# avaneev/avir

Measured on AMD Instinct MI355X. Metric: Mpixels/sec (output) for 4K->8K RGBA resize, higher is better.
Workload: dtype f32; 1 GPU; cfg3: 3840x2160->7680x4320 RGBA float32, avir::CImageResizer<>(16), k=0, default params, frame resident in HBM

## Files before the change

avir_amd/csrc/up2.hip:

```cpp

#include "plan.h"
#include "up2_chunks.h"
#include <algorithm>
#include <string.h>
#include <stdlib.h>
#include <stdio.h>
#include <type_traits>

namespace avirhip {

typedef float f4 __attribute__(( ext_vector_type( 4 )));
typedef float f2 __attribute__(( ext_vector_type( 2 )));
typedef unsigned u2 __attribute__(( ext_vector_type( 2 )));

#ifndef U2_TW
#define U2_TW 64
#endif
#define U2_NT ( U2_TW * 2 )
#ifndef U2_RB
#define U2_RB 8
#endif
#ifndef U2_HS
#define U2_HS 4
#endif
#define U2_SW ( U2_TW / 2 + 18 )
#define U2_CW ( U2_TW / 2 + 12 )

struct Up2Params
{
	const float* src; long src_ss; int sw, sh;
	int rmin, rmax;
	float* dst; long dst_ss; int dst_row0; int nw, nh;
	int srow_lo, srow_hi;
	int nstrips, chunk0, nchunks;
	int cq, nlong;
	void* ibase; int istride_b; int ich;
#ifdef U2_DBG
	int dbg;
	unsigned long long* clk;
#endif
	const float* coef;
};

typedef float f8 __attribute__(( ext_vector_type( 8 )));
typedef float f16 __attribute__(( ext_vector_type( 16 )));
#define U2_PAIRED 64

__device__ __forceinline__ f2 splat( const float c )
{
	f2 r; r.x = c; r.y = c; return( r );
}

struct Taps
{
	f16 a, b, c;
	f8 d;
	__device__ __forceinline__ f2 pr( const f16& v, int i ) const
		{ f2 r; r.x = v[ 2 * i ]; r.y = v[ 2 * i + 1 ]; return( r ); }
	__device__ __forceinline__ f2 f( int i ) const { return( pr( a, i )); }
	__device__ __forceinline__ f2 fe( int i ) const
		{ return( i < 4 ? pr( a, 4 + i ) : pr( b, i - 4 )); }
	__device__ __forceinline__ f2 fo( int i ) const
	{
		if( i < 8 ) return( pr( c, i ));
		f2 r; r.x = d[ 2 * ( i - 8 )]; r.y = d[ 2 * ( i - 8 ) + 1 ];
		return( r );
	}
};

__device__ __forceinline__ const float* sgpr_ptr( const float* p )
{
	const unsigned long long a = (unsigned long long) p;
	const unsigned lo = __builtin_amdgcn_readfirstlane( (unsigned) a );
	const unsigned hi = __builtin_amdgcn_readfirstlane( (unsigned) ( a >> 32 ));
	return( (const float*) (( (unsigned long long) hi << 32 ) | lo ));
}

__device__ __forceinline__ Taps load_taps( const float* p0 )
{
	const float* const p = sgpr_ptr( p0 );
	Taps t;
	asm volatile( "s_load_dwordx16 %0, %4, 0x0\n\t"
		"s_load_dwordx16 %1, %4, 0x40\n\t"
		"s_load_dwordx16 %2, %4, 0x80\n\t"
		"s_load_dwordx8 %3, %4, 0xc0\n\t"
		AVIRHIP_WAITCNT_LGKM( 0 )
		: "=&s"( t.a ), "=&s"( t.b ), "=&s"( t.c ), "=&s"( t.d )
		: "s"( p ) : "memory" );
	return( t );
}

struct TapsI
{
	f8 a;
	f4 b;
	__device__ __forceinline__ f2 fe( int i ) const
		{ return( splat( i < 8 ? a[ i ] : b[ i - 8 ])); }
};

__device__ __forceinline__ TapsI load_taps_i( const float* p0 )
{
	const float* const p = sgpr_ptr( p0 );
	TapsI t;
	asm volatile( "s_load_dwordx8 %0, %2, 0x10\n\t"
		"s_load_dwordx4 %1, %2, 0x30\n\t"
		AVIRHIP_WAITCNT_LGKM( 0 )
		: "=&s"( t.a ), "=&s"( t.b ) : "s"( p ) : "memory" );
	return( t );
}

struct TapsE
{
	f16 a;
	__device__ __forceinline__ f2 f( int i ) const { return( splat( a[ i ])); }
	__device__ __forceinline__ f2 fe( int i ) const { return( splat( a[ 4 + i ])); }
};

__device__ __forceinline__ TapsE load_taps_e( const float* p0 )
{
	const float* const p = sgpr_ptr( p0 );
	TapsE t;
	asm volatile( "s_load_dwordx16 %0, %1, 0x0\n\t"
		AVIRHIP_WAITCNT_LGKM( 0 )
		: "=&s"( t.a ) : "s"( p ) : "memory" );
	return( t );
}

__device__ __forceinline__ f4 load_f4( const float* p0 )
{
	const float* const p = sgpr_ptr( p0 );
	f4 t;
	asm volatile( "s_load_dwordx4 %0, %1, 0x0\n\t" AVIRHIP_WAITCNT_LGKM( 0 )
		: "=&s"( t ) : "s"( p ) : "memory" );
	return( t );
}

__device__ __forceinline__ f8 load_f8( const float* p0 )
{
	const float* const p = sgpr_ptr( p0 );
	f8 t;
	asm volatile( "s_load_dwordx8 %0, %1, 0x0\n\t" AVIRHIP_WAITCNT_LGKM( 0 )
		: "=&s"( t ) : "s"( p ) : "memory" );
	return( t );
}

__device__ __forceinline__ f4 tmul( const f2 t, const f4 v )
{
	const f2 lo = t * v.lo;
	const f2 hi = t * v.hi;
	return( __builtin_shufflevector( lo, hi, 0, 1, 2, 3 ));
}

__device__ __forceinline__ int fresh_tid( const int wave )
{
	int l;
	asm volatile( "v_mbcnt_lo_u32_b32 %0, -1, 0\n\t"
		"v_mbcnt_hi_u32_b32 %0, -1, %0" : "=v"( l ));
	return( l + wave * 64 );
}

__device__ __forceinline__ int clampi( int i, int hi )
{
	return( i < 0 ? 0 : ( i > hi ? hi : i ));
}

#if U2_TW == 32
#define U2_SYNC() __builtin_amdgcn_fence( __ATOMIC_RELEASE, "wavefront" ); \
	__builtin_amdgcn_wave_barrier(); \
	__builtin_amdgcn_fence( __ATOMIC_ACQUIRE, "wavefront" )
#else
#define U2_SYNC() do { AVIRHIP_BARRIER_DRAIN(); __syncthreads(); } while( 0 )

#define U2_PRIO_H 0
#define U2_PRIO_V 1

__device__ __forceinline__ void u2_setprio( const int p )
{
	if( p == 0 ) __builtin_amdgcn_s_setprio( 0 );
	else if( p == 1 ) __builtin_amdgcn_s_setprio( 1 );
	else if( p == 2 ) __builtin_amdgcn_s_setprio( 2 );
	else __builtin_amdgcn_s_setprio( 3 );
}
#endif

#ifdef U2_DBG
#define U2_ON( bit ) ( !( P.dbg & ( bit )))
#define U2_ABL_H1( k ) ( !( P.dbg & 16 ) || ( k ) < 2 || wave == 0 )
#define U2_ABL_TAIL() ( !( P.dbg & 32 ) || abl_tail == 0 )
#else
#define U2_ON( bit ) true
#define U2_ABL_H1( k ) true
#define U2_ABL_TAIL() true
#endif

#ifndef U2_STAUX
#define U2_STAUX 2
#endif

#ifndef U2_LDAUX
#define U2_LDAUX 0
#endif

#define U2_TPL ( U2_RB * ( U2_TW / 2 ) + 8 )

#ifndef U2_H2PB
#define U2_H2PB 4
#endif

template< bool VT, int IO = 0, int SRC = 0 >
__global__ void __launch_bounds__( U2_NT )
__attribute__(( amdgpu_waves_per_eu( 4, 4 ))) k_up2( const Up2Params P )
{
	static_assert( IO == 0 || VT, "the fused output stage lives in the VT form" );
	static_assert( SRC == 0 || VT, "raw sources live in the VT form" );
	constexpr int SESZ = SRC / 10;
	constexpr int SCH = SRC % 10;
	constexpr int PXB = ( SRC != 0 ? SESZ * SCH : 16 );
	constexpr int ESZ = ( IO == 1 || IO == 4 ? 1 : ( IO == 2 || IO == 5 ? 2 : 4 ));
	__shared__ __attribute__(( aligned( 16 ))) f4 sS[ U2_RB * U2_SW ];
	__shared__ __attribute__(( aligned( 16 ))) f4 sC[ U2_RB * U2_CW ];
	__shared__ __attribute__(( aligned( 16 ))) f4 sT[ U2_TPL * 2 - 8 ];

#ifdef U2_DBG
	const unsigned long long dbg_c0 = clock64();
	const unsigned long long dbg_w0 = wall_clock64();

	if( P.dbg & ( 2048 | 4096 ))
	{
		const int slot = ( P.dbg & 2048 ? (( blockIdx.x >> 8 ) & 1 ) * 4 :
			( blockIdx.x >> 8 ) & 7 );

		for( int i = 0; i < slot; i++ )
		{
			__builtin_amdgcn_s_sleep( 25 );
		}
	}
#endif
	const int nwg = gridDim.x;
	const int b = blockIdx.x;
	const int xcd = b & 7;
	const int qd = nwg >> 3;
	const int rm = nwg & 7;
	const int item = ( xcd < rm ? xcd * ( qd + 1 ) :
		rm * ( qd + 1 ) + ( xcd - rm ) * qd ) + ( b >> 3 );

	const int strip = item / P.nchunks;
	const int chunk = P.chunk0 + item - strip * P.nchunks;
	const int tid = threadIdx.x;
	const int hf = tid & 1;
	const int col = tid >> 1;

	const int qx0 = strip * ( U2_TW / 2 );
	const int qy0 = up2_chunk_first( chunk, P.cq, P.nlong );
	const int qy1 = min( qy0 + up2_chunk_rows( chunk, P.cq, P.nlong ),
		P.nh >> 1 );
	const int u0 = qy0 - 9;
	const int nsteps = qy1 - qy0 + 18;
	const int xo = qx0 * 2 + col;
	const int ylo = max( qy0 * 2, P.srow_lo );
	const int yhi = min( qy1 * 2, P.srow_hi );
	const bool xok = ( xo < P.nw );
	const bool strip_full = ( qx0 * 2 + U2_TW <= P.nw );
	const int dlane_b = ( xo * 4 + hf * 2 ) * 4;
	const int drow_b = ( IO != 0 ? P.istride_b :
		(int) P.dst_ss * 4 );
	const int srow_b = (int) P.src_ss * ( SRC != 0 ? 1 : 4 );

	const int ubase = max( u0, P.rmin );
	const char* const sbase = (const char*) P.src + (long) ubase * srow_b;
	const int rsh = ( SRC != 0 ? (int) ( (unsigned long long) sbase & 3 ) : 0 );
	const __amdgpu_buffer_rsrc_t rsrc = __builtin_amdgcn_make_buffer_rsrc(
		(void*) ( sbase - rsh ), 0, ( SRC != 0 ?
		( rsh + ( P.rmax - ubase ) * srow_b + P.sw * PXB + 3 ) & ~3 : 0x7fffffff ),
		0x00020000 );
	const __amdgpu_buffer_rsrc_t rdst = __builtin_amdgcn_make_buffer_rsrc(
		(void*) ( P.dst + (long) ( qy0 * 2 - P.dst_row0 ) * P.dst_ss ), 0,
		0x7fffffff, 0x00020000 );

	f2 tw[ 8 ];
	f2 cw[ VT ? 1 : 16 ];
	f2 ea[ VT ? 12 : 1 ];
	f2 oa[ VT ? 12 : 1 ];

#pragma unroll
	for( int i = 0; i < 8; i++ ) tw[ i ] = (f2) 0.0f;
#pragma unroll
	for( int i = 0; i < ( VT ? 1 : 16 ); i++ ) cw[ i ] = (f2) 0.0f;
#pragma unroll
	for( int i = 0; i < ( VT ? 12 : 1 ); i++ ) ea[ i ] = oa[ i ] = (f2) 0.0f;

	constexpr int RPI0 = U2_NT / U2_SW;
	constexpr int CN0 = U2_RB * U2_CW;
	unsigned pkA = 0;
	unsigned pkB = 0;
	unsigned pkC = 0;
	unsigned pkD = 0;
	int pvoff = -1;
	int dlv = 0;
	int dlv2 = 0;

	if constexpr( VT )
	{
		typedef __attribute__(( address_space( 3 ))) void* lp;
		auto la = []( const void* q ) -> unsigned
			{ return( (unsigned) (unsigned long long) (lp) q ); };

		{
			const int r = tid / U2_SW;
			const int sx = clampi( qx0 - 9 + ( tid - r * U2_SW ), P.sw - 1 );
			pvoff = ( tid < RPI0 * U2_SW ? r * srow_b + sx * PXB + rsh : -1 );
		}

		if constexpr( IO != 0 )
		{
			dlv = ( xo < P.nw && hf * 2 < P.ich ?
				( xo * P.ich + hf * 2 ) * ESZ : (int) 0x80000000u );
			dlv2 = ( xo < P.nw && hf * 2 + 1 < P.ich ?
				( xo * P.ich + hf * 2 + 1 ) * ESZ : (int) 0x80000000u );
		}
		else
		{
			dlv = ( xo < P.nw ? ( xo * 4 + hf * 2 ) * 4 : (int) 0x80000000u );
		}

		{
			constexpr int LS = ( U2_HS == 4 ? 2 : 1 );
			const int hr = ( tid >> 6 ) * 4 + (( tid >> ( 1 + LS )) & 3 );
			const int hq = (( tid >> ( 3 + LS )) & ( 8 / U2_HS - 1 )) * 4 * U2_HS +
				(( tid >> 1 ) & ( U2_HS - 1 ));

			pkA = la( (const f2*) &sC[ hr * U2_CW + hq ] + hf ) |
				( la( (const f2*) sT + ((( col & 1 ) * U2_TPL + ( col >> 1 )) * 2 +
				hf )) << 16 );
			pkD = la( &sC[ tid ]) |
				( la( (const f2*) &sT[ hr * ( U2_TW / 2 ) + hq ] + hf ) << 16 );
		}

		unsigned ha[ 3 ], hd = 0;
#pragma unroll
		for( int k = 0; k < 3; k++ )
		{
			const int i = min( tid + k * U2_NT, CN0 - 1 );
			const int r = (int) ((unsigned) i / U2_CW );
			ha[ k ] = la( &sS[ i + r * ( U2_SW - U2_CW )]);
			hd = la( &sC[ i ]);
		}

		pkB = ha[ 0 ] | ( ha[ 1 ] << 16 );
		pkC = ha[ 2 ] | ( hd << 16 );
		asm volatile( "" : "+v"( pkA ), "+v"( pkB ), "+v"( pkC ), "+v"( pkD ),
			"+v"( pvoff ), "+v"( dlv ));

		if constexpr( IO != 0 )
		{
			asm volatile( "" : "+v"( dlv2 ));
		}
	}

	typedef const __attribute__(( address_space( 3 ))) f4* lds_cf4;
	typedef __attribute__(( address_space( 3 ))) f4* lds_f4;
	typedef const __attribute__(( address_space( 3 ))) f2* lds_cf2;
	typedef __attribute__(( address_space( 3 ))) f2* lds_f2;
	auto lo16 = []( const unsigned v ) -> unsigned
	{
		unsigned r;
		asm volatile( "v_and_b32 %0, 0xffff, %1" : "=v"( r ) : "v"( v ));
		return( r );
	};
	auto hi16 = []( const unsigned v ) -> unsigned
	{
		unsigned r;
		asm volatile( "v_lshrrev_b32 %0, 16, %1" : "=v"( r ) : "v"( v ));
		return( r );
	};

	constexpr int RPI = U2_NT / U2_SW;
	constexpr int NDMA = U2_RB / RPI;
	static_assert( RPI >= 1 && U2_RB % RPI == 0, "S tile / DMA geometry" );

	typedef __attribute__(( address_space( 3 ))) void* ldsptr;
	const int wave = __builtin_amdgcn_readfirstlane( tid >> 6 );
	const int wave_b = wave * 1024;

	auto raw_off = [&]( const int k, const int ub ) -> int
	{
		if( ub >= P.rmin && ub + U2_RB <= P.rmax + 1 )
		{
			return( pvoff >= 0 ? pvoff + ( ub - ubase + k * RPI ) * srow_b : -1 );
		}

		const int tid = fresh_tid( wave );
		const int pr_r = tid / U2_SW;
		const int pr_sx = clampi( qx0 - 9 + ( tid - pr_r * U2_SW ), P.sw - 1 );
		const int sy = min( max( ub + k * RPI + pr_r, P.rmin ), P.rmax );

		return( tid < RPI * U2_SW ? ( sy - ubase ) * srow_b + pr_sx * PXB + rsh :
			-1 );
	};

	auto land_raw = [&]( const int ub )
	{
		typedef const __attribute__(( address_space( 3 ))) unsigned* lds_cu;
		unsigned d0[ NDMA ], d1[ NDMA ];
		int off[ NDMA ];
		const int lw = ( threadIdx.x & 63 ) * 4;
#pragma unroll
		for( int k = 0; k < NDMA; k++ )
		{
			off[ k ] = raw_off( k, ub );
			const char* const st = (const char*) sS + k * RPI * U2_SW * 16 +
				wave_b + lw;
			d0[ k ] = *(lds_cu) (const void*) st;
			d1[ k ] = *(lds_cu) (const void*) ( st + 256 );
		}

		asm volatile( "s_waitcnt lgkmcnt(0)" ::: "memory" );
#pragma unroll
		for( int k = 0; k < NDMA; k++ )
		{
			if( off[ k ] >= 0 )
			{
				const unsigned sh = (unsigned) off[ k ] & 3u;
				const unsigned lo = __builtin_amdgcn_alignbyte( d1[ k ], d0[ k ], sh );
				f4 px;

				if( SESZ == 1 )
				{
					px.x = (float) ( lo & 0xffu );
					px.y = (float) (( lo >> 8 ) & 0xffu );
					px.z = (float) (( lo >> 16 ) & 0xffu );
					px.w = ( SCH == 4 ? (float) ( lo >> 24 ) : 0.0f );
				}
				else
				{
					const unsigned hi = d1[ k ] >> ( sh * 8 );
					px.x = (float) ( lo & 0xffffu );
					px.y = (float) ( lo >> 16 );
					px.z = (float) ( hi & 0xffffu );
					px.w = ( SCH == 4 ? (float) ( hi >> 16 ) : 0.0f );
				}

				*(f4*) ((char*) sS + k * RPI * U2_SW * 16 + wave_b + lw * 4 ) = px;
			}
		}
	};

	auto prefetch = [&]( const int ub )
	{
		if constexpr( SRC != 0 )
		{
#pragma unroll
			for( int k = 0; k < NDMA; k++ )
			{
				const int o = raw_off( k, ub );

				if( o >= 0 )
				{
					const ldsptr q = (ldsptr) ((char*) sS + k * RPI * U2_SW * 16 +
						wave_b );
					__builtin_amdgcn_raw_ptr_buffer_load_lds( rsrc, q, 4, o & ~3,
						0, 0, U2_LDAUX );
					__builtin_amdgcn_raw_ptr_buffer_load_lds( rsrc,
						(ldsptr) ((char*) q + 256 ), 4, ( o & ~3 ) + 4, 0, 0,
						U2_LDAUX );
				}
			}

			return;
		}

		if( VT && ub >= P.rmin && ub + U2_RB <= P.rmax + 1 )
		{
			if( pvoff >= 0 )
			{
#pragma unroll
				for( int k = 0; k < NDMA; k++ )
				{
					__builtin_amdgcn_raw_ptr_buffer_load_lds( rsrc,
						(ldsptr) ((char*) sS + k * RPI * U2_SW * 16 + wave_b ),
						16, pvoff, ( ub - ubase + k * RPI ) * srow_b, 0,
						U2_LDAUX );
				}
			}

			return;
		}

		const int tid = ( VT ? fresh_tid( wave ) : (int) threadIdx.x );
		const int pr_r = tid / U2_SW;
		const int pr_sx = clampi( qx0 - 9 + ( tid - pr_r * U2_SW ), P.sw - 1 );
		const bool pr_on = ( tid < RPI * U2_SW );
		const int pr_voff = pr_r * srow_b + pr_sx * 16;

		if( !pr_on )
		{
			return;
		}

		if( ub >= P.rmin && ub + U2_RB <= P.rmax + 1 )
		{
#pragma unroll
			for( int k = 0; k < NDMA; k++ )
			{
				__builtin_amdgcn_raw_ptr_buffer_load_lds( rsrc,
					(ldsptr) ((char*) sS + k * RPI * U2_SW * 16 + wave_b ), 16,
					pr_voff, ( ub - ubase + k * RPI ) * srow_b, 0, U2_LDAUX );
			}
		}
		else
		{
#pragma unroll
			for( int k = 0; k < NDMA; k++ )
			{
				const int sy = min( max( ub + k * RPI + pr_r, P.rmin ), P.rmax );
				__builtin_amdgcn_raw_ptr_buffer_load_lds( rsrc,
					(ldsptr) ((char*) sS + k * RPI * U2_SW * 16 + wave_b ), 16,
					( sy - ubase ) * srow_b + pr_sx * 16, 0, 0, U2_LDAUX );
			}
		}
	};

	constexpr int CN = U2_RB * U2_CW;
	constexpr int NH1 = ( CN + U2_NT - 1 ) / U2_NT;
	constexpr int H1EVERY = U2_RB / NH1;
	static_assert( NH1 <= U2_RB, "H1 iterations must fit into the marching steps" );
	static_assert( !VT || ( NH1 == 3 && CN == CN0 && RPI == RPI0 ), "VT: packed H1 addresses" );

	auto h1_iter = [&]( const int k, const f2 ( &h )[ 4 ])
	{
		const int i = tid + k * U2_NT;

		if(( k + 1 ) * U2_NT <= CN || i < CN )
		{
			const int r = (int) ((unsigned) i / U2_CW );
			const f4* s = &sS[ i + r * ( U2_SW - U2_CW )];
			const f4 s0 = s[ 0 ], s1 = s[ 1 ], s2 = s[ 2 ], s3 = s[ 3 ];
			const f4 s4 = s[ 4 ], s5 = s[ 5 ], s6 = s[ 6 ];
			f4 a = tmul( h[ 0 ], s3 );
			a = a + tmul( h[ 1 ], s4 + s2 );
			a = a + tmul( h[ 2 ], s5 + s1 );
			a = a + tmul( h[ 3 ], s6 + s0 );
			sC[ i ] = a;
		}
	};

	auto h1_iter_p = [&]( const int k, const f2 ( &h )[ 4 ])
	{
		const unsigned sa = ( k == 0 ? lo16( pkB ) : k == 1 ? hi16( pkB ) :
			lo16( pkC ));
		const unsigned da = ( k == 2 ? hi16( pkC ) :
			lo16( pkD ) + k * U2_NT * 16 );
		const lds_cf4 s = (lds_cf4) (unsigned long long) sa;
		const f4 s0 = s[ 0 ], s1 = s[ 1 ], s2 = s[ 2 ], s3 = s[ 3 ];
		const f4 s4 = s[ 4 ], s5 = s[ 5 ], s6 = s[ 6 ];
		f4 a = tmul( h[ 0 ], s3 );
		a = a + tmul( h[ 1 ], s4 + s2 );
		a = a + tmul( h[ 2 ], s5 + s1 );
		a = a + tmul( h[ 3 ], s6 + s0 );
		*(lds_f4) (unsigned long long) da = a;
	};

	auto h2_phase = [&]()
	{
		if( VT && U2_ON( 2 ))
		{
			const TapsI H = load_taps_i( P.coef );
			const lds_cf2 c = (lds_cf2) (unsigned long long) lo16( pkA );
			const lds_f2 t0 = (lds_f2) (unsigned long long) hi16( pkD );
			constexpr int NP = 3 * U2_HS + 13;
			constexpr int PB = U2_H2PB;
			constexpr int NB = ( NP + PB - 1 ) / PB;
			f2 e[ 4 ], o[ 4 ];
			f2 w[ 2 ][ PB ];

#pragma unroll
			for( int i = 0; i < 4; i++ ) e[ i ] = o[ i ] = (f2) 0.0f;
#pragma unroll
			for( int k = 0; k < PB; k++ ) w[ 0 ][ k ] = c[ k * 2 ];

#pragma unroll
			for( int b = 0; b < NB; b++ )
			{
#pragma unroll
				for( int k = 0; k < PB; k++ )
				{
					if(( b + 1 ) * PB + k < NP )
					{
						w[ ( b + 1 ) & 1 ][ k ] = c[ (( b + 1 ) * PB + k ) * 2 ];
					}
				}

#pragma unroll
				for( int kk = 0; kk < PB; kk++ )
				{
					const int k = b * PB + kk;
#pragma unroll
					for( int t = 0; t < 12; t++ )
					{
						bool any = false;
#pragma unroll
						for( int i = 0; i < 4; i++ )
						{
							any |= ( k < NP && ( k - i * U2_HS == t ||
								12 - k + i * U2_HS == t ));
						}

						if( any )
						{
							const f2 pr = H.fe( t ) * w[ b & 1 ][ kk ];
#pragma unroll
							for( int i = 0; i < 4; i++ )
							{
								if( k - i * U2_HS == t ) e[ i ] = e[ i ] + pr;
								if( 12 - k + i * U2_HS == t ) o[ i ] = o[ i ] + pr;
							}
						}
					}
				}

				asm volatile( "" ::: "memory" );
#pragma unroll
				for( int i = 0; i < 4; i++ )
				{
					if( i * U2_HS < ( b + 1 ) * PB ) asm volatile( "" : "+v"( e[ i ]));
					if( i * U2_HS + 1 < ( b + 1 ) * PB ) asm volatile( "" : "+v"( o[ i ]));
				}

				__builtin_amdgcn_sched_barrier( 0 );
			}

#pragma unroll
			for( int i = 0; i < 4; i++ )
			{
				t0[ i * U2_HS * 2 ] = e[ i ];
				t0[ ( U2_TPL + i * U2_HS ) * 2 ] = o[ i ];
			}
		}
		else
		if( U2_ON( 2 ))
		{
			const Taps H = load_taps( P.coef + U2_PAIRED );
			const int tid = ( VT ? fresh_tid( wave ) : (int) threadIdx.x );
			const int qq = tid & ( U2_TW / 2 - 1 );

			for( int r = tid / ( U2_TW / 2 ); r < U2_RB;
				r += U2_NT / ( U2_TW / 2 ))
			{
				const f4* c = &sC[ r * U2_CW + qq ];
				f4 e = (f4) 0.0f;
				f4 o = (f4) 0.0f;
				f4 w[ 13 ];

				if( VT )
				{
#pragma unroll
					for( int t = 0; t < 5; t++ ) w[ t ] = c[ t ];
#pragma unroll
					for( int t = 0; t < 4; t++ )
					{
						e = e + tmul( H.fe( t ), w[ t ]);
						o = o + tmul( H.fo( t ), w[ t + 1 ]);
					}

					__builtin_amdgcn_sched_barrier( 0 );
#pragma unroll
					for( int t = 5; t < 9; t++ ) w[ t ] = c[ t ];
#pragma unroll
					for( int t = 4; t < 8; t++ )
					{
						e = e + tmul( H.fe( t ), w[ t ]);
						o = o + tmul( H.fo( t ), w[ t + 1 ]);
					}

					__builtin_amdgcn_sched_barrier( 0 );
#pragma unroll
					for( int t = 9; t < 13; t++ ) w[ t ] = c[ t ];
#pragma unroll
					for( int t = 8; t < 12; t++ )
					{
						e = e + tmul( H.fe( t ), w[ t ]);
						o = o + tmul( H.fo( t ), w[ t + 1 ]);
					}
				}
				else
				{
#pragma unroll
				for( int t = 0; t < 7; t++ ) w[ t ] = c[ t ];
#pragma unroll
				for( int t = 0; t < 6; t++ )
				{
					e = e + tmul( H.fe( t ), w[ t ]);
					o = o + tmul( H.fo( t ), w[ t + 1 ]);
				}

				__builtin_amdgcn_sched_barrier( 0 );
#pragma unroll
				for( int t = 7; t < 13; t++ ) w[ t ] = c[ t ];
#pragma unroll
				for( int t = 6; t < 12; t++ )
				{
					e = e + tmul( H.fe( t ), w[ t ]);
					o = o + tmul( H.fo( t ), w[ t + 1 ]);
				}
				}

				sT[ r * ( U2_TW / 2 ) + qq ] = e;
				sT[ U2_TPL + r * ( U2_TW / 2 ) + qq ] = o;
			}
		}

	};

	auto march = [&]( auto R0C, const int ub, const bool more,
		const bool more2 )
	{
		constexpr int R0 = decltype( R0C )::value;

		if( more && U2_ON( 8 ))
		{
			prefetch( ub + U2_RB );
		}

		u2_setprio( U2_PRIO_H );
		h2_phase();

		U2_SYNC();
		u2_setprio( U2_PRIO_V );

		const Taps V = load_taps( P.coef + U2_PAIRED + 64 );
		f2 hv[ 4 ];
		{
			const f8 HF = load_f8( P.coef + U2_PAIRED );
#pragma unroll
			for( int t = 0; t < 4; t++ )
			{
				asm volatile( "v_mov_b32 %0, %2\n\tv_mov_b32 %1, %3"
					: "=&v"( hv[ t ].x ), "=&v"( hv[ t ].y )
					: "s"( HF[ t * 2 ]), "s"( HF[ t * 2 + 1 ]));
			}
		}
		const int yb = ( ub - 9 ) * 2;
		int so = ( yb - qy0 * 2 ) * drow_b;

		const f2* sT2 = (const f2*) sT +
			((( col & 1 ) * U2_TPL + ( col >> 1 )) * 2 + hf );

		auto vsteps = [&]( auto FASTC )
		{
			constexpr bool FAST = decltype( FASTC )::value;
			tw[ R0 & 7 ] = sT2[ 0 ];
#pragma unroll
			for( int rr = 0; rr < U2_RB; rr++ )
			{
				const int g = R0 + rr;

				if( rr + 1 < U2_RB )
				{
					tw[ ( g + 1 ) & 7 ] = sT2[ ( rr + 1 ) * U2_TW ];
				}

				f2 c2 = V.f( 0 ) * tw[ ( g - 3 ) & 7 ];
				c2 = c2 + V.f( 1 ) * ( tw[ ( g - 2 ) & 7 ] +
					tw[ ( g - 4 ) & 7 ]);
				c2 = c2 + V.f( 2 ) * ( tw[ ( g - 1 ) & 7 ] +
					tw[ ( g - 5 ) & 7 ]);
				c2 = c2 + V.f( 3 ) * ( tw[ g & 7 ] + tw[ ( g - 6 ) & 7 ]);
				cw[ g & 15 ] = c2;

				const int y0 = yb + rr * 2;

				if(( FAST || ( y0 + 1 >= ylo && y0 < yhi )) && U2_ON( 4 ))
				{
					f2 e = (f2) 0.0f;
					f2 o = (f2) 0.0f;
#pragma unroll
					for( int t = 0; t < 12; t++ )
					{
						const f2 pe = V.fe( t ) * cw[ ( g - 12 + t ) & 15 ];
						const f2 po = V.fo( t ) * cw[ ( g - 11 + t ) & 15 ];
						__builtin_amdgcn_sched_barrier( 0 );
						e = e + pe;
						o = o + po;
						__builtin_amdgcn_sched_barrier( 0 );
					}

					if(( FAST || ( xok && y0 >= ylo )) &&
						( U2_ON( 1 ) || e.x == 1234.5f ))
					{
						__builtin_amdgcn_raw_buffer_store_b64(
							__builtin_bit_cast( u2, e ), rdst, dlane_b, so, U2_STAUX );
					}

					if(( FAST || ( xok && y0 + 1 < yhi )) &&
						( U2_ON( 1 ) || o.y == 1234.5f ))
					{
						__builtin_amdgcn_raw_buffer_store_b64(
							__builtin_bit_cast( u2, o ), rdst, dlane_b,
							so + drow_b, U2_STAUX );
					}
				}

				so += 2 * drow_b;

				if( rr % H1EVERY == 0 && rr / H1EVERY < NH1 && more &&
					U2_ON( 2 ))
				{
					h1_iter( rr / H1EVERY, hv );
				}
			}
		};

		if( strip_full && yb >= ylo && yb + 2 * U2_RB <= yhi )
		{
			vsteps( std::true_type() );
		}
		else
		{
			vsteps( std::false_type() );
		}

		U2_SYNC();
	};

	prefetch( u0 );

	if constexpr( SRC != 0 )
	{
		AVIRHIP_WAIT_VM( 0 );
		land_raw( u0 );
	}

	U2_SYNC();

	{
		const f4 HF = load_f4( P.coef );
		f2 hp[ 4 ];
#pragma unroll
		for( int t = 0; t < 4; t++ )
		{
			hp[ t ] = splat( HF[ t ]);
		}

#pragma unroll
		for( int k = 0; k < NH1; k++ )
		{
			h1_iter( k, hp );
		}
	}

	U2_SYNC();

	if constexpr( VT )
	{
		static_assert( !VT || U2_RB == 8, "VT marching period is 3 x 8 rows" );
#ifdef U2_DBG
		int abl_tail = 0;
#endif
		void* const dbase = ( IO != 0 ? (void*) ( (char*) P.ibase +
			(long) ( qy0 * 2 - P.dst_row0 ) * P.istride_b ) :
			(void*) ( P.dst + (long) ( qy0 * 2 - P.dst_row0 ) * P.dst_ss ));

		auto store_io = [&]( const f2 v, const __amdgpu_buffer_rsrc_t rs,
			const int soff )
		{
			if constexpr( IO == 3 )
			{
				const float v0 = v.x, v1 = v.y;
				__builtin_amdgcn_raw_buffer_store_b32( __float_as_uint( v0 ), rs,
					dlv, soff, U2_STAUX );
				__builtin_amdgcn_raw_buffer_store_b32( __float_as_uint( v1 ), rs,
					dlv2, soff, U2_STAUX );
			}
			else
			if constexpr( IO == 4 || IO == 5 )
			{
				constexpr int PKI = ( IO == 4 ? 255 : 65535 );
				const int q0 = min( max( (int) ( v.x + 0.5f ), 0 ), PKI );
				const int q1 = min( max( (int) ( v.y + 0.5f ), 0 ), PKI );

				if constexpr( IO == 4 )
				{
					__builtin_amdgcn_raw_buffer_store_b8( (unsigned char) q0, rs,
						dlv, soff, U2_STAUX );
					__builtin_amdgcn_raw_buffer_store_b8( (unsigned char) q1, rs,
						dlv2, soff, U2_STAUX );
				}
				else
				{
					__builtin_amdgcn_raw_buffer_store_b16( (unsigned short) q0, rs,
						dlv, soff, U2_STAUX );
					__builtin_amdgcn_raw_buffer_store_b16( (unsigned short) q1, rs,
						dlv2, soff, U2_STAUX );
				}
			}
			else
			{
				constexpr float PK = ( IO == 1 ? 255.0f : 65535.0f );
				float t0 = (float) (int) ( v.x + 0.5f );
				float t1 = (float) (int) ( v.y + 0.5f );
				t0 = fminf( fmaxf( t0, 0.0f ), PK );
				t1 = fminf( fmaxf( t1, 0.0f ), PK );
				t0 = avirhip_x86_round_fix( v.x, t0, PK );
				t1 = avirhip_x86_round_fix( v.y, t1, PK );

				if constexpr( IO == 1 )
				{
					__builtin_amdgcn_raw_buffer_store_b8(
						(unsigned char) (unsigned) t0, rs, dlv, soff, U2_STAUX );
					__builtin_amdgcn_raw_buffer_store_b8(
						(unsigned char) (unsigned) t1, rs, dlv2, soff, U2_STAUX );
				}
				else
				{
					__builtin_amdgcn_raw_buffer_store_b16(
						(unsigned short) (unsigned) t0, rs, dlv, soff, U2_STAUX );
					__builtin_amdgcn_raw_buffer_store_b16(
						(unsigned short) (unsigned) t1, rs, dlv2, soff, U2_STAUX );
				}
			}
		};

		auto vstep_t = [&]( auto R0C, auto MODEC, const int ub,
			const bool more )
		{
			constexpr int R0 = decltype( R0C )::value;
			constexpr int MODE = decltype( MODEC )::value;
			const TapsE V = load_taps_e( P.coef + 32 );
			f2 hv[ 4 ];
			{
				const f4 HF = load_f4( P.coef );
#pragma unroll
				for( int t = 0; t < 4; t++ )
				{
					hv[ t ] = splat( HF[ t ]);
				}
			}

			const int yb = ( ub - 9 ) * 2;
			int so = ( yb - qy0 * 2 ) * drow_b;
			const int dlane_v = dlv;
			const lds_cf2 sT2 = (lds_cf2) (unsigned long long) hi16( pkA );
			const int rlo = min( max( ylo - ( yb + 1 ), 0 ), 2 * U2_RB );
			const int rhi = min( max( yhi - ( yb + 1 ), 0 ), 2 * U2_RB );
			const unsigned rmask = __builtin_amdgcn_readfirstlane(
				(( 1u << rhi ) - 1u ) & ~(( 1u << rlo ) - 1u ));

			tw[ R0 & 7 ] = sT2[ 0 ];
#pragma unroll
			for( int rr = 0; rr < U2_RB; rr++ )
			{
				const int g = R0 + rr;

				if( rr + 1 < U2_RB )
				{
					tw[ ( g + 1 ) & 7 ] = sT2[ ( rr + 1 ) * U2_TW ];
				}

				f2 c2 = V.f( 0 ) * tw[ ( g - 3 ) & 7 ];
				c2 = c2 + V.f( 1 ) * ( tw[ ( g - 2 ) & 7 ] +
					tw[ ( g - 4 ) & 7 ]);
				c2 = c2 + V.f( 2 ) * ( tw[ ( g - 1 ) & 7 ] +
					tw[ ( g - 5 ) & 7 ]);
				c2 = c2 + V.f( 3 ) * ( tw[ g & 7 ] + tw[ ( g - 6 ) & 7 ]);

				if( U2_ON( 4 ))
				{
#pragma unroll
					for( int t = 0; t < 12; t += 2 )
					{
						const bool we0 = ( MODE != 2 || t <= g - 6 );
						const bool wo0 = ( MODE != 2 || t >= 18 - g );
						const bool we1 = ( MODE != 2 || t + 1 <= g - 6 );
						const bool wo1 = ( MODE != 2 || t + 1 >= 18 - g );
						f2 p0, p1;

						if( we0 || wo0 ) p0 = V.fe( t ) * c2;
						if( we1 || wo1 ) p1 = V.fe( t + 1 ) * c2;

						__builtin_amdgcn_sched_barrier( 0 );

						if( we0 )
						{
							f2& a = ea[ ( g + 3 - t + 24 ) % 12 ];
							a = ( t == 0 ? (f2) 0.0f : a ) + p0;
						}

						if( wo0 )
						{
							f2& a = oa[ ( g + 3 + t ) % 12 ];
							a = a + p0;
						}

						if( we1 )
						{
							f2& a = ea[ ( g + 2 - t + 24 ) % 12 ];
							a = a + p1;
						}

						if( wo1 )
						{
							f2& a = oa[ ( g + 4 + t ) % 12 ];
							a = ( t + 1 == 11 ? (f2) 0.0f : a ) + p1;
						}

						__builtin_amdgcn_sched_barrier( 0 );
					}

					asm volatile( "" : "+v"( ea[ 0 ]), "+v"( ea[ 1 ]),
						"+v"( ea[ 2 ]), "+v"( ea[ 3 ]), "+v"( ea[ 4 ]),
						"+v"( ea[ 5 ]), "+v"( ea[ 6 ]), "+v"( ea[ 7 ]),
						"+v"( ea[ 8 ]), "+v"( ea[ 9 ]), "+v"( ea[ 10 ]),
						"+v"( ea[ 11 ]));
					asm volatile( "" : "+v"( oa[ 0 ]), "+v"( oa[ 1 ]),
						"+v"( oa[ 2 ]), "+v"( oa[ 3 ]), "+v"( oa[ 4 ]),
						"+v"( oa[ 5 ]), "+v"( oa[ 6 ]), "+v"( oa[ 7 ]),
						"+v"( oa[ 8 ]), "+v"( oa[ 9 ]), "+v"( oa[ 10 ]),
						"+v"( oa[ 11 ]));

					const f2 od = oa[ ( g + 3 ) % 12 ];
					const f2 ed = ea[ ( g + 4 ) % 12 ];

					if( MODE != 2 || g >= 17 )
					{
						if constexpr( IO != 0 )
						{
							store_io( od, __builtin_amdgcn_make_buffer_rsrc(
								dbase, 0, ( rmask & ( 1u << ( 2 * rr )) ?
								0x7fffffff : 0 ), 0x00020000 ), so + drow_b );
							store_io( ed, __builtin_amdgcn_make_buffer_rsrc(
								dbase, 0, ( rmask & ( 2u << ( 2 * rr )) ?
								0x7fffffff : 0 ), 0x00020000 ), so + 2 * drow_b );
						}
						else
						{
						if( U2_ON( 1 ) || od.x == 1234.5f )
						{
							__builtin_amdgcn_raw_buffer_store_b64(
								__builtin_bit_cast( u2, od ),
								__builtin_amdgcn_make_buffer_rsrc( dbase, 0,
								( rmask & ( 1u << ( 2 * rr )) ? 0x7fffffff : 0 ),
								0x00020000 ), dlane_v, so + drow_b, U2_STAUX );
						}

						if( U2_ON( 1 ) || ed.y == 1234.5f )
						{
							__builtin_amdgcn_raw_buffer_store_b64(
								__builtin_bit_cast( u2, ed ),
								__builtin_amdgcn_make_buffer_rsrc( dbase, 0,
								( rmask & ( 2u << ( 2 * rr )) ? 0x7fffffff : 0 ),
								0x00020000 ), dlane_v, so + 2 * drow_b, U2_STAUX );
						}
						}
					}
				}

				so += 2 * drow_b;
				asm volatile( "" : "+s"( so ));

				if( rr % H1EVERY == 0 && rr / H1EVERY < NH1 && U2_ON( 2 ) &&
					U2_ABL_H1( rr / H1EVERY ) && U2_ABL_TAIL())
				{
					h1_iter_p( rr / H1EVERY, hv );
				}
			}
		};

		typedef std::integral_constant< int, 0 > I0;
		typedef std::integral_constant< int, 1 > I1;
		typedef std::integral_constant< int, 2 > I2;
		typedef std::integral_constant< int, 8 > I8;
		typedef std::integral_constant< int, 16 > I16;

		auto march_t = [&]( auto R0C, auto RAMPC, const int sb )
		{
			const int ub = u0 + sb;
			const bool more = ( sb + U2_RB < nsteps );
#ifdef U2_DBG
			const bool tail_h2 = (( P.dbg & 32 ) && sb + 2 * U2_RB >= nsteps &&
				nsteps > 6 * U2_RB );
			abl_tail = (( P.dbg & 32 ) && sb + 3 * U2_RB >= nsteps &&
				sb + U2_RB < nsteps && nsteps > 6 * U2_RB ? 1 : 0 );
#endif

			if( more && U2_ON( 8 ))
			{
				prefetch( ub + U2_RB );
			}

#ifdef U2_DBG
			u2_setprio( P.dbg & 1024 ? ( P.dbg >> 6 ) & 3 : U2_PRIO_H );

			if( !tail_h2 )
#else
			u2_setprio( U2_PRIO_H );
#endif
			h2_phase();

			if constexpr( SRC != 0 )
			{
				if( more )
				{
					AVIRHIP_WAIT_VM( 0 );
					land_raw( ub + U2_RB );
				}
			}

			U2_SYNC();
#ifdef U2_DBG
			u2_setprio( P.dbg & 1024 ? ( P.dbg >> 8 ) & 3 : U2_PRIO_V );
#else
			u2_setprio( U2_PRIO_V );
#endif

			if( decltype( RAMPC )::value )
			{
				vstep_t( R0C, I2(), ub, more );
			}
			else
			{
				vstep_t( R0C, I1(), ub, more );
			}

			U2_SYNC();
		};

		march_t( I0(), std::true_type(), 0 );
		march_t( I8(), std::true_type(), 8 );
		march_t( I16(), std::true_type(), 16 );

		for( int sb = 24; sb < nsteps; sb += 24 )
		{
			march_t( I0(), std::false_type(), sb );

			if( sb + 8 >= nsteps )
			{
				break;
			}

			march_t( I8(), std::false_type(), sb + 8 );

			if( sb + 16 >= nsteps )
			{
				break;
			}

			march_t( I16(), std::false_type(), sb + 16 );
		}
	}
	else
	{
		for( int sb = 0; sb < nsteps; sb += 16 )
		{
#if U2_RB == 16
			march( std::integral_constant< int, 0 >(), u0 + sb, sb + 16 < nsteps,
				sb + 32 < nsteps );
#else
			march( std::integral_constant< int, 0 >(), u0 + sb, sb + 8 < nsteps,
				sb + 16 < nsteps );

			if( sb + 8 >= nsteps )
			{
				break;
			}

			march( std::integral_constant< int, 8 >(), u0 + sb + 8,
				sb + 16 < nsteps, sb + 24 < nsteps );
#endif
		}
	}

#ifdef U2_DBG
	if( tid == 0 && P.clk != nullptr )
	{
		P.clk[ blockIdx.x * 4 ] = clock64() - dbg_c0;
		P.clk[ blockIdx.x * 4 + 1 ] = dbg_w0;
		P.clk[ blockIdx.x * 4 + 2 ] = wall_clock64();
		P.clk[ blockIdx.x * 4 + 3 ] =
			(unsigned) __builtin_amdgcn_s_getreg(( 31 << 11 ) | 4 ) |
			((unsigned long long) __builtin_amdgcn_s_getreg(( 31 << 11 ) | 20 ) << 32 );
	}
#endif
}


struct Up2Axis
{
	float f[ 4 ], fe[ 12 ], fo[ 12 ];
};

static bool match_axis( const LAxis& ax, Up2Axis& A )
{
	if( ax.ops.size() != 2 || ax.dst_len != ax.src_len * 2 )
	{
		return( false );
	}

	const LOp& a = ax.ops[ 0 ];
	const LOp& g = ax.ops[ 1 ];

	if( a.type != OP_FIR || a.view != VIEW_CLAMP || a.rf != 1 || a.lat != 3 ||
		a.e != 3 || a.in_len != ax.src_len || a.out_len != ax.src_len + 6 ||
		g.type != OP_GATHER || g.view != VIEW_ZS || g.maxtaps != 12 ||
		g.in_len != a.out_len || g.out_len != ax.dst_len )
	{
		return( false );
	}

	for( int i = 0; i < 4; i++ )
	{
		A.f[ i ] = a.h_flt[ i ];
	}

	for( int t = 0; t < 12; t++ )
	{
		A.fe[ t ] = g.h_coef[ t ];
		A.fo[ t ] = g.h_coef[ 12 + t ];
	}

	for( int j = 0; j < g.out_len; j++ )
	{
		const int q = j >> 1;
		const int st = ( j & 1 ? q - 2 : q - 3 );
		const float* cf = &g.h_coef[ (size_t) j * 12 ];
		const float* rf = ( j & 1 ? A.fo : A.fe );

		if( g.h_start[ j ] != st || g.h_ntaps[ j ] != 12 ||
			st + 11 > g.zs_mmax || memcmp( cf, rf, 12 * sizeof( float )) != 0 )
		{
			return( false );
		}
	}

	return( true );
}

struct Up2Data
{
	Up2Axis h, v;
	float* d_coef;
	bool vsym;
	bool hsym;
};

static bool up2_vt( const avirhip_plan* p, const Up2Data* D )
{
	static const bool novt = ( getenv( "AVIRHIP_UP2_NOVT" ) != nullptr );

	return( D != nullptr && U2_RB == 8 && D -> vsym && D -> hsym && !novt &&
		!( p -> variant & AVIRHIP_VARIANT_UP2_PLAIN_V ));
}

int up2_prepare( avirhip_plan* p )
{
	p -> up2 = nullptr;

	if( p -> is_lancir || p -> ch != 4 )
	{
		return( AVIRHIP_OK );
	}

	Up2Data* D = new Up2Data();

	if( match_axis( p -> h, D -> h ) && match_axis( p -> v, D -> v ))
	{
		float hc[ U2_PAIRED + 128 ] = { 0 };
		const Up2Axis* ax[ 2 ] = { &D -> h, &D -> v };

		for( int a = 0; a < 2; a++ )
		{
			float* o = hc + a * 32;
			memcpy( o, ax[ a ] -> f, 4 * sizeof( float ));
			memcpy( o + 4, ax[ a ] -> fe, 12 * sizeof( float ));
			memcpy( o + 16, ax[ a ] -> fo, 12 * sizeof( float ));
			o = hc + U2_PAIRED + a * 64;

			for( int i = 0; i < 4; i++ )
			{
				o[ 2 * i ] = o[ 2 * i + 1 ] = ax[ a ] -> f[ i ];
			}

			for( int t = 0; t < 12; t++ )
			{
				o[ 8 + 2 * t ] = o[ 9 + 2 * t ] = ax[ a ] -> fe[ t ];
				o[ 32 + 2 * t ] = o[ 33 + 2 * t ] = ax[ a ] -> fo[ t ];
			}
		}

		void* q = nullptr;
		AVIRHIP_HIPCHECK( hipMalloc( &q, sizeof( hc )));
		p -> allocs.push_back( q );
		AVIRHIP_HIPCHECK( hipMemcpy( q, hc, sizeof( hc ),
			hipMemcpyHostToDevice ));
		D -> d_coef = (float*) q;
		D -> vsym = true;
		D -> hsym = true;

		for( int t = 0; t < 12; t++ )
		{
			D -> vsym &= ( memcmp( &D -> v.fo[ t ], &D -> v.fe[ 11 - t ],
				sizeof( float )) == 0 );
			D -> hsym &= ( memcmp( &D -> h.fo[ t ], &D -> h.fe[ 11 - t ],
				sizeof( float )) == 0 );
		}

		p -> up2 = D;
		p -> fused_ok |= 4;
		p -> auto_path = 4;
	}
	else
	{
		delete D;
	}

	return( AVIRHIP_OK );
}

void up2_release( avirhip_plan* p )
{
	delete (Up2Data*) p -> up2;
	p -> up2 = nullptr;
}

bool up2_stores_io( const avirhip_plan* p )
{
	const Up2Data* D = (const Up2Data*) p -> up2;

	return( up2_vt( p, D ) && !p -> gamma &&
		p -> dither == AVIRHIP_DITHER_DEF &&
		(( p -> out_type == AVIRHIP_U8 && p -> tr_mul == 1.0 &&
		p -> pk_out == 255.0 ) ||
		( p -> out_type == AVIRHIP_U16 && p -> tr_mul == 1.0 &&
		p -> pk_out == 65535.0 ) ||
		( p -> out_type == AVIRHIP_F32 && p -> io_ch < 4 )));
}

bool up2_takes_window( const avirhip_plan* p, const void* src, const void* dst )
{
	return( p -> up2 != nullptr && !p -> is_lancir && p -> ch == 4 &&
		p -> io_ch == 4 && p -> in_type == AVIRHIP_F32 &&
		p -> out_type == AVIRHIP_F32 && !p -> gamma &&
		( (uintptr_t) src & 15 ) == 0 && ( (uintptr_t) dst & 7 ) == 0 &&
		( p -> src_stride & 3 ) == 0 &&
		(long) p -> src_stride * 4 < ( 1L << 22 ) &&
		(long) p -> new_w * 16 < ( 1L << 22 ));
}

int up2_run( avirhip_plan* p, const float* src, long src_stride, float* dst,
	int row0, int row1, hipStream_t st, SrcWindow win, const ImageRef* rawimg,
	void* iout )
{
	const void* const raw = ( rawimg != nullptr ? rawimg -> ptr : nullptr );
	const long raw_stride = ( rawimg != nullptr ? rawimg -> stride : 0 );
	const Up2Data* D = (const Up2Data*) p -> up2;
	int io = 0;

	if( iout != nullptr )
	{
		const bool vt = up2_vt( p, D );

		io = ( p -> out_type == AVIRHIP_U8 && p -> tr_mul == 1.0 &&
			p -> pk_out == 255.0 ? 1 :
			( p -> out_type == AVIRHIP_U16 && p -> tr_mul == 1.0 &&
			p -> pk_out == 65535.0 && ( (uintptr_t) iout & 1 ) == 0 ? 2 :
			( p -> out_type == AVIRHIP_F32 && p -> io_ch < 4 &&
			( (uintptr_t) iout & 3 ) == 0 ? 3 : 0 )));

		if( !vt || io == 0 || p -> dither != AVIRHIP_DITHER_DEF || p -> gamma )
		{
			return( 1 );
		}

		if(( io == 1 || io == 2 ) && ( p -> in_type == AVIRHIP_U8 ||
			p -> in_type == AVIRHIP_U16 ))
		{
			io += 3;
		}

	}

	int srck = 0;

	if( raw != nullptr )
	{
		const int esz = ( p -> in_type == AVIRHIP_U8 ? 1 : 2 );
		const long sb = raw_stride * esz;

		if(( io != 4 && io != 5 ) || ( p -> io_ch != 3 && p -> io_ch != 4 ) ||
			win.rows > 0 || ( (uintptr_t) raw & ( esz - 1 )) ||
			( esz == 2 && p -> io_ch == 4 && (( (uintptr_t) raw | sb ) & 3 )) ||
			sb >= ( 1L << 22 ) || getenv( "AVIRHIP_UP2_NO_RAW" ) != nullptr )
		{
			return( 1 );
		}

		srck = esz * 10 + p -> io_ch;
		src = (const float*) raw;
		src_stride = sb;
	}

	if( D == nullptr || ( srck == 0 && (( (uintptr_t) src & 15 ) ||
		( src_stride & 3 ))) || ( io == 0 && ( (uintptr_t) dst & 7 )))
	{
		return( 1 );
	}

	if( row1 <= row0 )
	{
		return( AVIRHIP_OK );
	}

	if(( srck == 0 && (long) src_stride * 4 >= ( 1L << 22 )) ||
		(long) p -> new_w * 16 >= ( 1L << 22 ))
	{
		return( 1 );
	}

	Up2Params P;
	P.src = src; P.src_ss = src_stride; P.sw = p -> src_w; P.sh = p -> src_h;
	P.rmin = ( win.rows > 0 ? win.first : 0 );
	P.rmax = ( win.rows > 0 ? win.first + win.rows : p -> src_h ) - 1;
	P.dst = dst; P.dst_ss = (long) p -> new_w * 4; P.dst_row0 = row0;
	P.nw = p -> new_w; P.nh = p -> new_h;
	P.srow_lo = row0; P.srow_hi = row1;
	P.nstrips = ( p -> new_w + U2_TW - 1 ) / U2_TW;
	P.ibase = iout; P.ich = p -> io_ch;
	P.istride_b = p -> new_w * p -> io_ch * ( io == 1 || io == 4 ? 1 :
		( io == 2 || io == 5 ? 2 : 4 ));

	const int rows = ( row1 - 1 ) / 2 - row0 / 2 + 1;
	Up2Split sp = up2_split_choose( rows, P.nstrips );

	const char* ecq = getenv( "AVIRHIP_UP2_CQ" );
	const char* enc = getenv( "AVIRHIP_UP2_NCHUNKS" );

	if( ecq != nullptr && atoi( ecq ) >= 6 )
	{
		sp.cq = (( atoi( ecq ) + 18 + U2_RB - 1 ) / U2_RB ) * U2_RB - 18;
		sp.nlong = 0;
	}
	else
	if( enc != nullptr && atoi( enc ) >= 1 &&
		up2_split_n( rows, atoi( enc ), 4 ).n != 0 )
	{
		sp = up2_split_n( rows, atoi( enc ), 4 );
	}

	P.cq = sp.cq;
	P.nlong = sp.nlong;
	P.chunk0 = up2_chunk_of( row0 / 2, P.cq, P.nlong );
	const int chunk1 = up2_chunk_of(( row1 - 1 ) / 2, P.cq, P.nlong );

	P.coef = D -> d_coef;
#ifdef U2_DBG
	P.dbg = ( getenv( "AVIRHIP_UP2_DBG" ) != nullptr ?
		atoi( getenv( "AVIRHIP_UP2_DBG" )) : 0 );
	static unsigned long long* dclk = nullptr;
	static int dclk_calls = 0;

	if( dclk == nullptr )
	{
		(void) hipMalloc( &dclk, 8192 * 32 );
	}

	P.clk = dclk;
#endif

	P.nchunks = chunk1 - P.chunk0 + 1;
	const int items = P.nstrips * P.nchunks;

	if( getenv( "AVIRHIP_VERBOSE" ) != nullptr )
	{
		int nb = -1;
		(void) hipOccupancyMaxActiveBlocksPerMultiprocessor( &nb,
			(const void*) k_up2< false, 0 >, U2_NT, 0 );
		fprintf( stderr, "k_up2: %d items (strips %d, cq %d, nlong %d), "
			"occupancy API %d workgroups/CU\n", items, P.nstrips, P.cq,
			P.nlong, nb );
	}

	const char* pad = getenv( "AVIRHIP_UP2_LDSPAD" );
	const int ldspad = ( pad != nullptr ? atoi( pad ) : 0 );
	if( srck != 0 )
	{
#define U2_RAW( IOK, SK ) hipLaunchKernelGGL(( k_up2< U2_RB == 8, \
	U2_RB == 8 ? IOK : 0, U2_RB == 8 ? SK : 0 > ), dim3( items ), \
	dim3( U2_NT ), ldspad, st, P )
		if( io == 4 )
		{
			switch( srck )
			{
				case 13: U2_RAW( 4, 13 ); break;
				case 14: U2_RAW( 4, 14 ); break;
				case 23: U2_RAW( 4, 23 ); break;
				default: U2_RAW( 4, 24 ); break;
			}
		}
		else
		{
			switch( srck )
			{
				case 13: U2_RAW( 5, 13 ); break;
				case 14: U2_RAW( 5, 14 ); break;
				case 23: U2_RAW( 5, 23 ); break;
				default: U2_RAW( 5, 24 ); break;
			}
		}
#undef U2_RAW
	}
	else
	if( io != 0 )
	{
		switch( io )
		{
			case 1: hipLaunchKernelGGL(( k_up2< U2_RB == 8, U2_RB == 8 ? 1 : 0 > ),
				dim3( items ), dim3( U2_NT ), ldspad, st, P ); break;
			case 2: hipLaunchKernelGGL(( k_up2< U2_RB == 8, U2_RB == 8 ? 2 : 0 > ),
				dim3( items ), dim3( U2_NT ), ldspad, st, P ); break;
			case 3: hipLaunchKernelGGL(( k_up2< U2_RB == 8, U2_RB == 8 ? 3 : 0 > ),
				dim3( items ), dim3( U2_NT ), ldspad, st, P ); break;
			case 4: hipLaunchKernelGGL(( k_up2< U2_RB == 8, U2_RB == 8 ? 4 : 0 > ),
				dim3( items ), dim3( U2_NT ), ldspad, st, P ); break;
			default: hipLaunchKernelGGL(( k_up2< U2_RB == 8, U2_RB == 8 ? 5 : 0 > ),
				dim3( items ), dim3( U2_NT ), ldspad, st, P ); break;
		}
	}
	else
	if( up2_vt( p, D ))
	{
		hipLaunchKernelGGL(( k_up2< U2_RB == 8, 0 > ), dim3( items ), dim3( U2_NT ),
			ldspad, st, P );
	}
	else
	{
		hipLaunchKernelGGL(( k_up2< false, 0 > ), dim3( items ), dim3( U2_NT ),
			ldspad, st, P );
	}
	AVIRHIP_HIPCHECK( hipGetLastError() );
#ifdef U2_DBG
	if( ++dclk_calls == 60 && items <= 8192 )
	{
		std::vector< unsigned long long > h( items * 4 );
		(void) hipStreamSynchronize( st );
		(void) hipMemcpy( h.data(), dclk, items * 32, hipMemcpyDeviceToHost );
		double sc = 0.0, sw = 0.0, mx = 0.0;
		unsigned long long t0 = ~0ULL, t1 = 0;

		for( int i = 0; i < items; i++ )
		{
			const double w = (double) ( h[ i * 4 + 2 ] - h[ i * 4 + 1 ]);
			sc += (double) h[ i * 4 ];
			sw += w;
			mx = std::max( mx, w );
			t0 = std::min( t0, h[ i * 4 + 1 ]);
			t1 = std::max( t1, h[ i * 4 + 2 ]);
		}

		fprintf( stderr, "k_up2 clocks: mean item %.0f shader cycles, %.2f us "
			"(max %.2f us, first start to last end %.2f us) => %.3f GHz\n",
			sc / items, sw / items / 100.0, mx / 100.0,
			(double) ( t1 - t0 ) / 100.0, sc / sw * 0.1 );

		const char* dump = getenv( "AVIRHIP_UP2_CLKDUMP" );

		if( dump != nullptr )
		{
			FILE* f = fopen( dump, "w" );

			for( int i = 0; f != nullptr && i < items; i++ )
			{
				fprintf( f, "%d %llu %llu %llu %llx\n", i, h[ i * 4 ],
					h[ i * 4 + 1 ] - t0, h[ i * 4 + 2 ] - t0, h[ i * 4 + 3 ]);
			}

			if( f != nullptr ) fclose( f );
		}
	}
#endif
	return( AVIRHIP_OK );
}

}
```

Baseline: 254,800 Mpixels/s.

## Remap H1 horizontal pass to per-thread runs sharing a sliding window

Replaces the per-pixel H1 filter, where each thread read 7 f4 source pixels from LDS for one output, with a run-based mapping. Each thread handles a half-channel pair along a contiguous run of pixels and reuses an 8-sample window across two outputs per slice. A new header supplies a compile-time thread-to-task map built to limit LDS bank conflicts. The aim is to cut LDS read traffic and address registers (pkC is dropped), at the cost of uneven run lengths across the two waves and a fixed geometry enforced by static asserts.

```diff
diff --git a/avir_amd/csrc/up2.hip b/avir_amd/csrc/up2.hip
--- a/avir_amd/csrc/up2.hip
+++ b/avir_amd/csrc/up2.hip
@@ -1,6 +1,7 @@
 
 #include "plan.h"
 #include "up2_chunks.h"
+#include "up2_h1map.h"
 #include <algorithm>
 #include <string.h>
 #include <stdlib.h>
@@ -293,7 +294,6 @@
 	constexpr int CN0 = U2_RB * U2_CW;
 	unsigned pkA = 0;
 	unsigned pkB = 0;
-	unsigned pkC = 0;
 	unsigned pkD = 0;
 	int pvoff = -1;
 	int dlv = 0;
@@ -332,23 +332,17 @@
 			pkA = la( (const f2*) &sC[ hr * U2_CW + hq ] + hf ) |
 				( la( (const f2*) sT + ((( col & 1 ) * U2_TPL + ( col >> 1 )) * 2 +
 				hf )) << 16 );
-			pkD = la( &sC[ tid ]) |
-				( la( (const f2*) &sT[ hr * ( U2_TW / 2 ) + hq ] + hf ) << 16 );
-		}
-
-		unsigned ha[ 3 ], hd = 0;
-#pragma unroll
-		for( int k = 0; k < 3; k++ )
-		{
-			const int i = min( tid + k * U2_NT, CN0 - 1 );
-			const int r = (int) ((unsigned) i / U2_CW );
-			ha[ k ] = la( &sS[ i + r * ( U2_SW - U2_CW )]);
-			hd = la( &sC[ i ]);
-		}
-
-		pkB = ha[ 0 ] | ( ha[ 1 ] << 16 );
-		pkC = ha[ 2 ] | ( hd << 16 );
-		asm volatile( "" : "+v"( pkA ), "+v"( pkB ), "+v"( pkC ), "+v"( pkD ),
+			pkD = la( (const f2*) &sT[ hr * ( U2_TW / 2 ) + hq ] + hf );
+		}
+
+		{
+			const Up2H1Task t = up2_h1_task( tid );
+
+			pkB = ( la( sS ) + up2_h1_src( t )) |
+				(( la( sC ) + up2_h1_dst( t )) << 16 );
+		}
+
+		asm volatile( "" : "+v"( pkA ), "+v"( pkB ), "+v"( pkD ),
 			"+v"( pvoff ), "+v"( dlv ));
 
 		if constexpr( IO != 0 )
@@ -357,8 +351,6 @@
 		}
 	}
 
-	typedef const __attribute__(( address_space( 3 ))) f4* lds_cf4;
-	typedef __attribute__(( address_space( 3 ))) f4* lds_f4;
 	typedef const __attribute__(( address_space( 3 ))) f2* lds_cf2;
 	typedef __attribute__(( address_space( 3 ))) f2* lds_f2;
 	auto lo16 = []( const unsigned v ) -> unsigned
@@ -524,7 +516,9 @@
 	constexpr int NH1 = ( CN + U2_NT - 1 ) / U2_NT;
 	constexpr int H1EVERY = U2_RB / NH1;
 	static_assert( NH1 <= U2_RB, "H1 iterations must fit into the marching steps" );
-	static_assert( !VT || ( NH1 == 3 && CN == CN0 && RPI == RPI0 ), "VT: packed H1 addresses" );
+	static_assert( !VT || ( NH1 == 3 && 2 * NH1 == UP2_H1_LONG &&
+		UP2_H1_SHORT == UP2_H1_LONG - 1 && CN == CN0 && RPI == RPI0 ),
+		"VT: H1 runs of 6 and 5 pixels in three slices of two" );
 
 	auto h1_iter = [&]( const int k, const f2 ( &h )[ 4 ])
 	{
@@ -544,20 +538,33 @@
 		}
 	};
 
-	auto h1_iter_p = [&]( const int k, const f2 ( &h )[ 4 ])
-	{
-		const unsigned sa = ( k == 0 ? lo16( pkB ) : k == 1 ? hi16( pkB ) :
-			lo16( pkC ));
-		const unsigned da = ( k == 2 ? hi16( pkC ) :
-			lo16( pkD ) + k * U2_NT * 16 );
-		const lds_cf4 s = (lds_cf4) (unsigned long long) sa;
-		const f4 s0 = s[ 0 ], s1 = s[ 1 ], s2 = s[ 2 ], s3 = s[ 3 ];
-		const f4 s4 = s[ 4 ], s5 = s[ 5 ], s6 = s[ 6 ];
-		f4 a = tmul( h[ 0 ], s3 );
-		a = a + tmul( h[ 1 ], s4 + s2 );
-		a = a + tmul( h[ 2 ], s5 + s1 );
-		a = a + tmul( h[ 3 ], s6 + s0 );
-		*(lds_f4) (unsigned long long) da = a;
+	auto h1_run = [&]( const int k, const f2 ( &h )[ 4 ])
+	{
+		const unsigned back = ( k == NH1 - 1 ? wave * 16 : 0 );
+		const lds_cf2 s = (lds_cf2) (unsigned long long)
+			( lo16( pkB ) + k * 32 - back );
+		const lds_f2 d = (lds_f2) (unsigned long long)
+			( hi16( pkB ) + k * 32 - back );
+		f2 w[ 8 ];
+#pragma unroll
+		for( int i = 0; i < 8; i++ ) w[ i ] = s[ i * 2 ];
+
+#ifdef U2_H1PINV
+		asm volatile( "" : "+v"( w[ 0 ]), "+v"( w[ 1 ]), "+v"( w[ 2 ]),
+			"+v"( w[ 3 ]), "+v"( w[ 4 ]), "+v"( w[ 5 ]), "+v"( w[ 6 ]),
+			"+v"( w[ 7 ]) :: "memory" );
+#else
+		asm volatile( "" ::: "memory" );
+#endif
+#pragma unroll
+		for( int j = 0; j < 2; j++ )
+		{
+			f2 a = h[ 0 ] * w[ j + 3 ];
+			a = a + h[ 1 ] * ( w[ j + 4 ] + w[ j + 2 ]);
+			a = a + h[ 2 ] * ( w[ j + 5 ] + w[ j + 1 ]);
+			a = a + h[ 3 ] * ( w[ j + 6 ] + w[ j ]);
+			d[ j * 2 ] = a;
+		}
 	};
 
 	auto h2_phase = [&]()
@@ -566,7 +573,7 @@
 		{
 			const TapsI H = load_taps_i( P.coef );
 			const lds_cf2 c = (lds_cf2) (unsigned long long) lo16( pkA );
-			const lds_f2 t0 = (lds_f2) (unsigned long long) hi16( pkD );
+			const lds_f2 t0 = (lds_f2) (unsigned long long) pkD;
 			constexpr int NP = 3 * U2_HS + 13;
 			constexpr int PB = U2_H2PB;
 			constexpr int NB = ( NP + PB - 1 ) / PB;
@@ -844,7 +851,8 @@
 #pragma unroll
 		for( int k = 0; k < NH1; k++ )
 		{
-			h1_iter( k, hp );
+			if constexpr( VT ) h1_run( k, hp );
+			else h1_iter( k, hp );
 		}
 	}
 
@@ -1060,7 +1068,7 @@
 				if( rr % H1EVERY == 0 && rr / H1EVERY < NH1 && U2_ON( 2 ) &&
 					U2_ABL_H1( rr / H1EVERY ) && U2_ABL_TAIL())
 				{
-					h1_iter_p( rr / H1EVERY, hv );
+					h1_run( rr / H1EVERY, hv );
 				}
 			}
 		};
diff --git a/avir_amd/csrc/up2_h1map.h b/avir_amd/csrc/up2_h1map.h
--- /dev/null
+++ b/avir_amd/csrc/up2_h1map.h
@@ -0,0 +1,116 @@
+
+#ifndef AVIRHIP_UP2_H1MAP_H
+#define AVIRHIP_UP2_H1MAP_H
+
+#ifndef U2_TW
+#define U2_TW 64
+#endif
+#ifndef U2_RB
+#define U2_RB 8
+#endif
+#ifndef U2_NT
+#define U2_NT ( U2_TW * 2 )
+#endif
+#ifndef U2_SW
+#define U2_SW ( U2_TW / 2 + 18 )
+#endif
+#ifndef U2_CW
+#define U2_CW ( U2_TW / 2 + 12 )
+#endif
+
+namespace avirhip {
+
+#define UP2_H1_LONG ( U2_CW / 8 + 1 )
+#define UP2_H1_SHORT ( U2_CW / 8 )
+#define UP2_H1_SPITCH ( U2_SW * 16 )
+#define UP2_H1_CPITCH ( U2_CW * 16 )
+
+static_assert( U2_NT == 128 && U2_RB == 8, "H1 map: 2 waves, 8 rows" );
+static_assert( 4 * ( UP2_H1_LONG + UP2_H1_SHORT ) == U2_CW,
+	"H1 map: a row is four long and four short runs" );
+static_assert( U2_RB * 2 * 8 == U2_NT, "H1 map: one task per thread" );
+
+struct Up2H1Task
+{
+	int row;
+	int half;
+	int col;
+	int len;
+};
+
+constexpr Up2H1Task up2_h1_task( const int tid )
+{
+	const int wave = tid >> 6;
+	const int l = tid & 63;
+	const int run = (( l >> 3 ) & 1 ) | ((( l >> 5 ) & 1 ) << 1 );
+
+	return( Up2H1Task{ (( l >> 1 ) & 3 ) | ((( l >> 4 ) & 1 ) << 2 ), l & 1,
+		run * ( UP2_H1_LONG + UP2_H1_SHORT ) + wave * UP2_H1_LONG,
+		wave == 0 ? UP2_H1_LONG : UP2_H1_SHORT });
+}
+
+constexpr int up2_h1_src( const Up2H1Task t )
+{
+	return( t.row * UP2_H1_SPITCH + t.col * 16 + t.half * 8 );
+}
+
+constexpr int up2_h1_dst( const Up2H1Task t )
+{
+	return( t.row * UP2_H1_CPITCH + t.col * 16 + t.half * 8 );
+}
+
+constexpr int up2_h1_conflict( const bool write, const int group,
+	const int nbank8 )
+{
+	int worst = 0;
+
+	for( int wave = 0; wave < 2; wave++ )
+	{
+		const int len = ( wave == 0 ? UP2_H1_LONG : UP2_H1_SHORT );
+		const int npos = ( write ? len : len + 6 );
+
+		for( int k = 0; k < npos; k++ )
+		{
+			for( int g = 0; g < 64; g += group )
+			{
+				for( int a = 0; a < group; a++ )
+				{
+					const Up2H1Task ta = up2_h1_task( wave * 64 + g + a );
+					const int ua = (( write ? up2_h1_dst( ta ) :
+						up2_h1_src( ta )) + k * 16 ) / 8;
+					int n = 1;
+
+					for( int b = 0; b < group; b++ )
+					{
+						const Up2H1Task tb = up2_h1_task( wave * 64 + g + b );
+						const int ub = (( write ? up2_h1_dst( tb ) :
+							up2_h1_src( tb )) + k * 16 ) / 8;
+						bool first = true;
+
+						for( int c = 0; c < b; c++ )
+						{
+							const Up2H1Task tc = up2_h1_task( wave * 64 + g + c );
+							const int uc = (( write ? up2_h1_dst( tc ) :
+								up2_h1_src( tc )) + k * 16 ) / 8;
+							first = first && ( uc != ub );
+						}
+
+						n += ( ub != ua && first &&
+							( ub - ua ) % nbank8 == 0 );
+					}
+
+					worst = ( n > worst ? n : worst );
+				}
+			}
+		}
+	}
+
+	return( worst );
+}
+
+#define UP2_H1_READ_DEGREE 1
+#define UP2_H1_WRITE_DEGREE 2
+
+}
+
+#endif
```

Result: no change. 256,000 Mpixels/s, median of 6 (+0.5%).
